# jgkellymit/GENIE-SMEM

Hardware: AMD Instinct MI355X
Metric: query-bases/sec SMEM discovery, 100kb ref x 150bp reads; bit-exact SMEM set (higher is better)
Workload: dtype u8/int32 (2-bit packed bases, int32 SA rows; f64 only in the RMI predict)

## Files before the change

### genie-smem_amd/csrc/kernels.hip

```cpp
#include <hip/hip_runtime.h>

#include <algorithm>
#include <cstdio>
#include <cstdlib>
#include <mutex>
#include <string>
#include <unordered_map>

#include "genie_internal.h"

namespace genie {

namespace {

constexpr int kWave = 64;

__device__ __forceinline__ int rfl(int v) { return __builtin_amdgcn_readfirstlane(v); }
__device__ __forceinline__ void set_wave_priority(int i)
{
    switch (i & 3) {
    case 0: __builtin_amdgcn_s_setprio(0); break;
    case 1: __builtin_amdgcn_s_setprio(1); break;
    case 2: __builtin_amdgcn_s_setprio(2); break;
    default: __builtin_amdgcn_s_setprio(3); break;
// ... 647 lines not shown
    int64_t at = 0;
    template <class T> void take(T *&piece, int64_t bytes)
    {
        piece = base ? reinterpret_cast<T *>(base + at) : nullptr;
        at += ws_align(bytes);
    }
};

template <class F>
inline long long pass_size(long long lo, long long total, F fits)
{
    long long hi = std::max(lo, total);
    while (lo < hi) {
        const long long mid = lo + (hi - lo + 1) / 2;
        if (fits(mid)) lo = mid; else hi = mid - 1;
    }
    return std::min(lo, total);
}

inline int64_t block_sums_bytes(int64_t N) { return (N / 16 + 3) * 8; }

inline int64_t workspace_layout(uint8_t *base, int64_t N, const Geometry &g, Workspace *ws, int64_t vlens_n = 0)
{
    Carver c{base};
    c.take(ws->fwd, N * (int64_t)g.fwd_stride);
    c.take(ws->qp, N * (int64_t)g.qp_stride * 16);
    c.take(ws->status, N * 4);
    c.take(ws->kj, N * (int64_t)g.kj_row * (g.wide ? 4 : 2));
    c.take(ws->counts, N * 4);
    c.take(ws->scan_tmp, block_sums_bytes(N));
    c.take(ws->vlens, vlens_n * 4);
    return c.at + 256;
}

inline int carve_workspace(void *d_ws, int64_t ws_bytes, int64_t N, const Geometry &g, Workspace *ws, int64_t vlens_n = 0)
{
    if (!d_ws || ws_bytes < workspace_layout(static_cast<uint8_t *>(d_ws), N, g, ws, vlens_n) || (reinterpret_cast<uintptr_t>(d_ws) & 255) != 0)
        return GENIE_E_CAPACITY;
    return GENIE_OK;
}

constexpr long long kLongTwoLaneReads = 32768;

struct FindRequest : FindBatch {
    int32_t *counts = nullptr, *slots = nullptr;
    int32_t cap = 0;
    int64_t *offsets = nullptr;
    int32_t *rows = nullptr;
    int64_t cap_rows = 0;
    bool packed = false;
    int row_bytes = 8;
    uint8_t *counts8 = nullptr, *status8 = nullptr;
    int64_t *escapes = nullptr;
    int64_t cap_escapes = 0;
    bool both = false;

    explicit FindRequest(const FindBatch &b) : FindBatch(b) {}
};

constexpr int kLdsBytes = 160 * 1024;
std::mutex g_lds_mu;
std::unordered_map<const void *, int> g_lds_limit;

template <class Kernel>
int allow_large_lds(Kernel k)
{
    const void *fn = reinterpret_cast<const void *>(k);
    int limit;
    {
        std::lock_guard<std::mutex> lk(g_lds_mu);
        auto it = g_lds_limit.find(fn);
        if (it == g_lds_limit.end()) {
            hipFuncAttributes attr;
            HIP_TRY(hipFuncGetAttributes(&attr, fn));
            it = g_lds_limit.emplace(fn, kLdsBytes - (int)attr.sharedSizeBytes).first;
        }
        limit = it->second;
    }
    HIP_TRY(hipFuncSetAttribute(fn, hipFuncAttributeMaxDynamicSharedMemorySize, limit));
    return GENIE_OK;
}

template <class Kernel, class... Args>
int launch_match_table(Kernel km, const Geometry &g, hipStream_t s, Args... args)
{
    if (int rc = allow_large_lds(km)) return rc;
    LAUNCH(km, dim3(g.grid), dim3(g.block), g.lds, s, args...);
    return GENIE_OK;
}

template <int MODE, bool WIDE>
int launch_pipeline(const genie_index *ix, const Geometry &g, const FindRequest &r, const Workspace &ws, hipStream_t s)
{
    int32_t *st = r.status ? r.status : ws.status;
    int32_t *cnt = r.counts ? r.counts : ws.counts;
    const bool c16 = (ix->dev.flags & kFlagCompactTable) != 0;
    const long long mtab_bytes = table_bytes(ix);
    const int cus = ix->num_cus > 0 ? ix->num_cus : 256;
    const int max_len = std::max(g.max_len, 1);
    const int long_flags = ix->opt_search_all | ix->opt_scheduling << 16, flags = long_flags | ix->opt_debug << 8;
    if (ix->ev_search_begin) HIP_TRY(hipEventRecord((hipEvent_t)ix->ev_search_begin, s));
    int rc;
    if (WIDE && r.both)
        rc = launch_match_table(c16 ? match_table_long_both_kernel<true> : match_table_long_both_kernel<false>, g, s, ix->dev,
                                (int)MODE, r.reads, r.lens, (long long)r.N, r.stride, r.fixed_len, reinterpret_cast<uint8_t *>(ws.fwd),
                                g.fwd_stride, ws.qp, g.qp_recs, st, max_len, mtab_bytes, long_flags, cus, ws.vlens);
    else if (WIDE)
        rc = launch_match_table(c16 ? match_table_long_kernel<true> : match_table_long_kernel<false>, g, s, ix->dev, (int)MODE,
                                r.reads, r.lens, (long long)r.N, r.stride, r.fixed_len, reinterpret_cast<uint8_t *>(ws.fwd),
                                g.fwd_stride, ws.qp, g.qp_recs, st, max_len, mtab_bytes, long_flags, cus);
    else if (r.both)
        rc = launch_match_table(c16 ? (g.wps == 4 ? match_table_both_kernel<4, true> : match_table_both_kernel<6, true>)
                                    : (g.wps == 4 ? match_table_both_kernel<4, false> : match_table_both_kernel<8, false>),
                                g, s, ix->dev, (int)MODE, r.reads, r.lens, (long long)r.N, r.stride, r.fixed_len,
                                reinterpret_cast<uint8_t *>(ws.fwd), g.fwd_stride, ws.qp, g.qp_recs, g.qp_stride, st, g.grp,
                                max_len, mtab_bytes, flags, cus, ws.vlens);
    else
        rc = launch_match_table(r.packed ? (c16 ? (g.wps == 4 ? match_table_kernel<4, true, true> : match_table_kernel<6, true, true>)
                                                : (g.wps == 4 ? match_table_kernel<4, false, true> : match_table_kernel<8, false, true>))
                                         : (c16 ? (g.wps == 4 ? match_table_kernel<4, true, false> : match_table_kernel<6, true, false>)
                                                : (g.wps == 4 ? match_table_kernel<4, false, false> : match_table_kernel<8, false, false>)),
                                g, s, ix->dev, (int)MODE, r.reads, r.lens, (long long)r.N, r.stride, r.fixed_len,
                                reinterpret_cast<uint8_t *>(ws.fwd), g.fwd_stride, ws.qp, g.qp_recs, g.qp_stride, st, g.grp,
                                max_len, mtab_bytes, flags, cus);
    if (rc) return rc;
    if (ix->ev_search_end) HIP_TRY(hipEventRecord((hipEvent_t)ix->ev_search_end, s));
    if (ix->opt_search_only) return GENIE_W_SEARCH_ONLY;
    const long long N = r.N;
    const int32_t *lens = r.both && r.lens ? ws.vlens : r.lens;
    uint8_t *head = WIDE ? ws.kj : reinterpret_cast<uint8_t *>(ws.qp) + g.qp_recs * 16;
    const int head_stride = WIDE ? g.kj_row * 4 : g.qp_stride * 16;
    const int tb = 256;
    int reads_per_block = tb;
    unsigned long long *bsums = r.offsets ? reinterpret_cast<unsigned long long *>(ws.scan_tmp) : nullptr;
    if (WIDE) {
        const int lanes = N >= kLongTwoLaneReads ? 2 : 16;
        auto kl = lanes == 2 ? traverse_long_kernel<MODE, 2, 8> : traverse_long_kernel<MODE, 16, 1>;
        LAUNCH(kl, dim3((unsigned)((N + tb / lanes - 1) / (tb / lanes))), dim3(tb), lanes == 2 ? (tb / lanes) * kLongRowBytes : 0, s, lens,
               N, r.fixed_len, r.min_len, ws.fwd, g.fwd_stride, cnt, reinterpret_cast<uint32_t *>(ws.kj),
               g.kj_row, r.offsets ? g.kj_row : r.cap, st, bsums);
        reads_per_block = tb / lanes;
    } else {
        auto kb = traverse_kernel<MODE>;
        const int lds_b = tb * g.fwd_lds;
        if ((rc = allow_large_lds(kb))) return rc;
        LAUNCH(kb, dim3((unsigned)((N + tb - 1) / tb)), dim3(tb), lds_b, s, ix->dev, lens, N,
               r.fixed_len, r.min_len, ws.fwd, g.fwd_stride, g.fwd_lds, cnt, ws.kj, g.kj_row, head, head_stride,
               r.offsets ? g.kj_row : r.cap, st, bsums, r.counts8, r.status8);
    }
    int block_shift = 0;
    while ((1 << block_shift) < reads_per_block) block_shift++;
    if (r.offsets)
        LAUNCH(scan_block_sums_kernel, dim3(1), dim3(kScanBlock), 0, s, bsums, (N + reads_per_block - 1) / reads_per_block);
    long long grid_c = (long long)cus * (32 / kIvWaves);
    const long long need_c = (N + kIvWaves * 4 * kIvUnroll - 1) / (kIvWaves * 4 * kIvUnroll);
    if (grid_c > need_c) grid_c = need_c;
    RowEscapes esc{nullptr, nullptr, 0};
    const int sched_c = ((ix->opt_scheduling >> 2) & 1) | cus << 8;
    if (r.packed) {
        esc.count = reinterpret_cast<unsigned long long *>(r.offsets) + 1;
        esc.list = reinterpret_cast<long long *>(r.escapes);
        esc.cap = r.cap_escapes;
        HIP_TRY(hipMemsetAsync(r.offsets, 0, 16, s));
    }
    auto kc = r.packed ? (r.row_bytes == 6 ? (c16 ? interval_kernel<true, false, true, 2> : interval_kernel<true, false, false, 2>)
                                           : (c16 ? interval_kernel<true, false, true, 1> : interval_kernel<true, false, false, 1>))
            : r.offsets ? (c16 ? interval_kernel<true, WIDE, true> : interval_kernel<true, WIDE, false>)
                        : (c16 ? interval_kernel<false, WIDE, true> : interval_kernel<false, WIDE, false>);
    LAUNCH(kc, dim3((unsigned)grid_c), dim3(kIvWaves * kWave), 0, s, ix->dev, N, ws.kj, g.kj_row, head, head_stride, ws.qp,
           g.qp_stride, r.offsets ? reinterpret_cast<void *>(r.rows) : reinterpret_cast<void *>(r.slots), r.offsets ? 0 : r.cap,
           reinterpret_cast<long long *>(r.offsets), r.offsets ? (long long)r.cap_rows : 0ll, bsums, r.offsets ? cnt : nullptr,
           r.offsets ? block_shift : 0, esc, sched_c);
    return GENIE_OK;
}

template <int MODE>
int launch_find_mode(const genie_index *ix, const Geometry &g, const FindRequest &r, hipStream_t s)
{
    Workspace ws;
    int rc = carve_workspace(r.ws, r.ws_bytes, r.N, g, &ws, r.both ? r.N : 0);
    if (rc) return rc;
    if (g.wide) return launch_pipeline<MODE, true>(ix, g, r, ws, s);
    return launch_pipeline<MODE, false>(ix, g, r, ws, s);
}

}

void set_hip_error(const char *what, int code)
{
    std::lock_guard<std::mutex> lk(g_err_mu);
    g_err = std::string(what) + ": " + hipGetErrorString((hipError_t)code);
}

const char *last_hip_error()
{
    std::lock_guard<std::mutex> lk(g_err_mu);
    return g_err.c_str();
}

int find_smems_geometry(const genie_index *ix, int32_t mode, int32_t max_len, int32_t *grid, int32_t *block,
                        int32_t *lds_bytes)
{
    Geometry g;
    int rc = plan_find_smems(ix, mode, max_len, 1ll << 40, &g);
    if (rc) return rc;
    if (grid) *grid = g.grid;
    if (block) *block = g.block;
    if (lds_bytes) *lds_bytes = g.lds;
    return GENIE_OK;
}

int search_kernel_name(const genie_index *ix, int32_t mode, int32_t max_len, char *buf, int32_t cap)
{
    Geometry g;
    int rc = plan_find_smems(ix, mode, max_len, 1ll << 40, &g);
    if (rc) return rc;
    const std::string c16 = (ix->dev.flags & kFlagCompactTable) ? "true" : "false";
    const std::string name = g.wide ? "match_table_long_kernel<" + c16 + ">"
                                    : "match_table_kernel<" + std::to_string(g.wps) + ", " + c16 + ", false>";
    if (!buf || cap < (int)name.size() + 1) return GENIE_E_CAPACITY;
    memcpy(buf, name.c_str(), name.size() + 1);
    return GENIE_OK;
}

int64_t find_smems_workspace_bytes(int64_t N, int32_t max_len)
{
    Geometry g;
    shape_for(max_len, &g);
    Workspace ws;
    return workspace_layout(nullptr, N, g, &ws);
}

void find_smems_workspace_rows(int32_t max_len, int32_t out[4])
{
    Geometry g;
    shape_for(max_len, &g);
    out[0] = g.fwd_stride;
    out[1] = g.qp_recs;
    out[2] = 0;
    out[3] = g.kj_row * (g.wide ? 4 : 2);
}

static int launch_find_any(const genie_index *ix, int32_t mode, const FindRequest &r, void *stream)
{
    hipStream_t s = (hipStream_t)stream;
    if (r.N == 0) {
        if (r.offsets) HIP_TRY(hipMemsetAsync(r.offsets, 0, r.packed ? 16 : 8, s));
        return GENIE_OK;
    }
    Geometry g;
    int rc = plan_find_smems(ix, mode, r.fixed_len, r.N, &g);
    if (rc) return rc;
    switch (mode) {
    case GENIE_MODE_BWA: return launch_find_mode<GENIE_MODE_BWA>(ix, g, r, s);
    case GENIE_MODE_LUT: return launch_find_mode<GENIE_MODE_LUT>(ix, g, r, s);
    case GENIE_MODE_RMI: return launch_find_mode<GENIE_MODE_RMI>(ix, g, r, s);
    }
    return GENIE_E_INVALID;
}

int launch_find_smems(const genie_index *ix, int32_t mode, const FindBatch &b, int32_t *d_counts, int32_t *d_slots, int32_t cap,
                      void *stream)
{
    FindRequest r(b);
    r.counts = d_counts;
    r.slots = d_slots;
    r.cap = cap;
    return launch_find_any(ix, mode, r, stream);
}

int launch_find_smems_csr(const genie_index *ix, int32_t mode, const FindBatch &b, int64_t *d_offsets, int32_t *d_rows,
                          int64_t out_cap_rows, void *stream)
{
    FindRequest r(b);
    r.offsets = d_offsets;
    r.rows = d_rows;
    r.cap_rows = out_cap_rows;
    return launch_find_any(ix, mode, r, stream);
}

int64_t find_smems_both_workspace_bytes(int64_t N, int32_t max_len)
{
    Geometry g;
    shape_for(max_len, &g);
    Workspace ws;
    return workspace_layout(nullptr, 2 * N, g, &ws, 2 * N);
}

int launch_find_smems_both(const genie_index *ix, int32_t mode, const FindBatch &b, int64_t *d_offsets, int32_t *d_rows,
                           int64_t out_cap_rows, void *stream)
{
    FindRequest r(b);
    r.N = 2 * b.N;
    r.offsets = d_offsets;
    r.rows = d_rows;
    r.cap_rows = out_cap_rows;
    r.both = true;
    return launch_find_any(ix, mode, r, stream);
}

int launch_find_smems_packed(const genie_index *ix, int32_t mode, const FindBatch &b, uint8_t *d_counts8, uint8_t *d_status8,
                             void *d_rows8, int64_t out_cap_rows, int64_t *d_totals, int64_t *d_escapes, int64_t cap_escapes,
                             void *stream, int row_bytes)
{
    FindRequest r(b);
    r.offsets = d_totals;
    r.rows = reinterpret_cast<int32_t *>(d_rows8);
    r.cap_rows = out_cap_rows;
    r.packed = true;
    r.row_bytes = row_bytes;
    r.counts8 = d_counts8;
    r.status8 = d_status8;
    r.escapes = d_escapes;
    r.cap_escapes = cap_escapes;
    return launch_find_any(ix, mode, r, stream);
}

int launch_sa_interval(const genie_index *ix, const uint8_t *d_pats, const int32_t *d_lens, int64_t N, int32_t stride,
                       int32_t fixed_len, int32_t *d_out, void *stream)
{
// ... 218 lines not shown
```

### genie-smem_amd/csrc/short_read_kernel.inc

```

template <bool WIDE>
struct ReadTraits {
    typedef uint8_t fwd_t;
    static constexpr int kj_bits = 16, kj_shift = 8;
};
template <>
struct ReadTraits<true> {
    typedef uint16_t fwd_t;
    static constexpr int kj_bits = 32, kj_shift = 16;
};


typedef unsigned short kb_us2 __attribute__((ext_vector_type(2)));
__device__ __forceinline__ uint32_t kb_pk_max(uint32_t a, uint32_t b)
{
    return __builtin_bit_cast(uint32_t, __builtin_elementwise_max(__builtin_bit_cast(kb_us2, a), __builtin_bit_cast(kb_us2, b)));
}

constexpr int kPairHeadWords = 4;

__device__ __forceinline__ int block_exclusive_scan(int v, int &total)
{
    __shared__ int wave_total[16];
    const int lane = threadIdx.x & (kWave - 1), wave = threadIdx.x >> 6;
// ... 175 lines not shown
    constexpr int kShift = ReadTraits<true>::kj_shift;
    const int lane = threadIdx.x & (kWave - 1), sub = lane & (G - 1);
    const long long r = (long long)blockIdx.x * (blockDim.x / G) + (threadIdx.x / G);
    const bool valid = r < N;
    int st = valid ? status[r] : GENIE_READ_OK;
    const int L = valid ? (lens ? lens[r] : fixed_len) : 0;
    const uint16_t *fw = reinterpret_cast<const uint16_t *>(fwd_in + (valid ? r : 0) * (long long)fwd_stride);
    uint32_t *row = kj_out + (valid ? r : 0) * (long long)kj_stride;
    int i = 0, cnt = 0;
    uint32_t mine = 0;
    bool go = valid && st == GENIE_READ_OK && L > 0;
    int kprev = -1;
    while (__any(go)) {
        uint32_t best = 0;
        int top = i;
        bool more = go;
        if (V == 8) {
            int ctop = i >> 3;
            const uint32_t reach = ((uint32_t)i << 16) | 0xFFFFu;
            bool first = true;
            const int need_lo = (kprev + 1) & ~7;
            const bool fits = go && i - need_lo < kLongWin;
            const bool reload = fits && !(need_lo >= wb && i < wb + kLongWin);
            if (__any(reload)) {
                if (reload) {
                    wb = need_lo;
                    uint4 t[kLongWin / 8 / G];
#pragma unroll
                    for (int u = 0; u < kLongWin / 8 / G; u++) {
                        const int c = (wb >> 3) + sub + G * u;
                        t[u] = c < row_chunks ? *reinterpret_cast<const uint4 *>(fw + 8 * c) : make_uint4(0, 0, 0, 0);
                    }
#pragma unroll
                    for (int u = 0; u < kLongWin / 8 / G; u++) *reinterpret_cast<uint4 *>(wrow + 16 * (sub + G * u)) = t[u];
                }
                wave_lds_fence();
            }
            while (__any(more)) {
                const int c = ctop - sub;
                const bool inb = more && c >= 0;
                uint4 q = make_uint4(0, 0, 0, 0);
                if (inb) {
                    if (fits && 8 * c >= wb) q = *reinterpret_cast<const uint4 *>(wrow + 2 * (8 * c - wb));
                    else q = *reinterpret_cast<const uint4 *>(fw + 8 * c);
                }
                uint32_t qd[4] = {q.x, q.y, q.z, q.w};
                if (first) {
                    const int jmax = (sub == 0) ? (i & 7) : 7;
#pragma unroll
                    for (int d = 0; d < 4; d++) qd[d] &= jmax >= 2 * d + 1 ? 0xFFFFFFFFu : (jmax >= 2 * d ? 0x0000FFFFu : 0u);
                    first = false;
                }
                const uint32_t c0 = (uint32_t)(0xFFFF - 8 * c) - ((uint32_t)(8 * c) << 16);
                uint32_t kmax = 0;
#pragma unroll
                for (int j = 0; j < 8; j++) {
                    const uint32_t vh = (j & 1) ? (qd[j >> 1] & 0xFFFF0000u) : (qd[j >> 1] << 16);
                    const uint32_t key = vh > reach ? vh + (c0 - (uint32_t)j * 0x10001u) : 0u;
                    kmax = max(kmax, key);
                }
                best = max(best, group_max<G>(kmax));
                const bool low = inb && (qd[0] << 16) > reach;
                ctop -= G;
                more = more && ((__ballot(low) >> (lane | (G - 1))) & 1ull);
            }
        }
        while (V == 1 && __any(more)) {
            const int k = top - sub;
            const bool in = more && k > kprev;
            const int v = in ? (int)fw[k] : 0;
            const bool covers = in && v > i;
            const uint32_t key = covers ? ((uint32_t)(v - k) << 16) | (uint32_t)(0xFFFF - k) : 0u;
            best = max(best, group_max<G>(key));
            top -= G;
            more = more && ((__ballot(covers) >> (lane | (G - 1))) & 1ull);
        }
        if (go) {
            const int blen = (int)(best >> 16), bk = 0xFFFF - (int)(best & 0xFFFFu);
            if (blen == 0) { st = GENIE_READ_ABSENT_BASE; go = false; }
            else {
                if (MODE != GENIE_MODE_BWA || blen >= min_len) {
                    const int s_ = cnt + 1;
                    if (sub == (s_ & (G - 1))) mine = (uint32_t)(bk | ((bk + blen) << kShift));
                    if ((s_ & (G - 1)) == G - 1) {
                        const int idx = (s_ & ~(G - 1)) + sub;
                        if (idx > 0) row[idx] = mine;
                    }
                    cnt++;
                }
                kprev = bk;
                i = bk + blen;
                go = i < L;
            }
        }
    }
    if (valid) {
        if (st != GENIE_READ_OK) cnt = 0;
        else {
            const int idx = ((cnt + 1) & ~(G - 1)) + sub;
            if (((cnt + 1) & (G - 1)) != 0 && idx >= 1 && idx <= cnt) row[idx] = mine;
            if (cnt > cap) st = GENIE_READ_OVERFLOW;
        }
        if (sub == 0) {
            row[0] = (uint32_t)cnt;
            status[r] = st;
        }
    }
    if (block_sums) {
        int total;
        const int before = block_exclusive_scan(valid && sub == 0 ? cnt : 0, total);
        if (valid && sub == 0) counts[r] = before;
        if (threadIdx.x == 0) block_sums[blockIdx.x] = (unsigned long long)total;
    } else if (valid && sub == 0) {
        counts[r] = cnt;
    }
}

constexpr int kIvWaves = 8;
constexpr int kIvUnroll = 1;
constexpr int kIvList = 128;

struct RowEscapes {
    unsigned long long *count;
    long long *list;
    long long cap;
};
template <int COUT>
__device__ __forceinline__ void emit_row(void *out, long long idx, int k, int j, int lo, int hi, const RowEscapes &esc)
{
    if (COUT == 0) {
        store_nt(reinterpret_cast<int4 *>(out) + idx, make_uint4((uint32_t)k, (uint32_t)j, (uint32_t)lo, (uint32_t)hi));
        return;
    }
    constexpr uint32_t kTop = COUT == 1 ? 0xFFFFu : 0xFFu;
    uint32_t span = (uint32_t)(hi - lo);
    if (span >= kTop) {
        const unsigned long long slot = atomicAdd(esc.count, 1ull);
        if ((long long)slot < esc.cap) {
            esc.list[2 * slot] = idx;
            esc.list[2 * slot + 1] = hi;
        }
        span = kTop;
    }
    if (COUT == 1) {
        reinterpret_cast<uint2 *>(out)[idx] = make_uint2((uint32_t)k | (uint32_t)j << 8 | span << 16, (uint32_t)lo);
    } else {
        uint16_t *o = reinterpret_cast<uint16_t *>(out) + 3 * idx;
        o[0] = (uint16_t)((uint32_t)k | (uint32_t)j << 8);
        o[1] = (uint16_t)lo;
        o[2] = (uint16_t)(((uint32_t)lo >> 16) | span << 8);
    }
}

template <bool CSR, bool WIDE, bool C16, int COUT = 0>
__global__ void __launch_bounds__(kIvWaves * 64, 8) interval_kernel(DevIndex ix, long long N,
                                                                    const void *__restrict__ kj_in, int kj_stride,
                                                                    const uint8_t *__restrict__ head_in, int head_stride,
                                                                    const RefRec *__restrict__ qp_in, int qp_stride,
                                                                    void *__restrict__ out, int cap,
                                                                    long long *__restrict__ offsets, long long out_cap,
                                                                    const unsigned long long *__restrict__ block_base,
                                                                    const int32_t *__restrict__ before_in_block, int block_shift,
                                                                    RowEscapes esc, int sched)
{
    __shared__ int4 lists[kIvWaves][kIvList];
    typedef typename std::conditional<WIDE, uint32_t, uint16_t>::type kj_t;
    typedef typename std::conditional<WIDE, QRecs, QPlain>::type QIn;
    constexpr int kHeadEntries = kPairHeadWords * 8 / (int)sizeof(kj_t);
    const int lane = threadIdx.x & (kWave - 1);
    const int wave = rfl((int)(threadIdx.x >> 6));
    const int sub = lane & 15;
    const int P2 = ix.P2;
    const __amdgpu_buffer_rsrc_t ov =
        __builtin_amdgcn_make_buffer_rsrc(const_cast<MatchOv16 *>(ix.ov), 0, ix.ov_entries * (int)sizeof(MatchOv16), 0x00020000);
    int4 *list = lists[wave];
    int nlist = 0;
    auto search_list = [&](int o, int n) {
        if (lane < n) {
            const int4 en = list[o + lane];
            const int k = en.w & 0xFFFF, j = (int)((uint32_t)en.w >> 16);
            const QIn qp{reinterpret_cast<decltype(QIn::p)>(qp_in + (long long)en.z * qp_stride)};
            const int2 iv = sa_interval(ix, ix.dir, qp, k, j - k);
            emit_row<COUT>(out, ((long long)en.y << 32) | (uint32_t)en.x, k, j, iv.x, iv.y, esc);
        }
    };
    constexpr int U = kIvUnroll;
    const long long step = (long long)gridDim.x * kIvWaves * 4 * U;
    const bool rotate = !(sched & 1);
    const int round_of_block = (int)(blockIdx.x / (uint32_t)(sched >> 8));
    int it = round_of_block;
    for (long long r0 = ((long long)blockIdx.x * kIvWaves + wave) * 4 * U; r0 < N; r0 += step, it++) {
        if (rotate) set_wave_priority(it);
        long long r[U], base[U];
        int c[U];
        bool more = false;
#pragma unroll
        for (int u = 0; u < U; u++) {
            r[u] = r0 + 4 * u + (lane >> 4);
            const bool have = r[u] < N;
            if (!have) r[u] = 0;
            c[u] = have ? (int)reinterpret_cast<const kj_t *>(head_in + r[u] * (long long)head_stride)[0] : 0;
            base[u] = CSR ? (have ? (long long)block_base[r[u] >> block_shift] + before_in_block[r[u]] : 0) : r[u] * (long long)cap;
            if (CSR && have && sub == 0) {
                if (!COUT) offsets[r[u]] = base[u];
                if (r[u] == N - 1) offsets[COUT ? 0 : N] = base[u] + c[u];
            }
            if (!CSR) c[u] = c[u] < cap ? c[u] : cap;
            more |= c[u] > 0;
        }
        for (int t0 = 0; __any(more); t0 += 16) {
            const int t = t0 + sub;
            uint32_t e[U];
            uint64_t w[U];
            int4 ra[U], rb[U];
            bool act[U];
            more = false;
#pragma unroll
            for (int u = 0; u < U; u++) {
                act[u] = t < c[u] && (!CSR || base[u] + t < out_cap);
                more |= t0 + 16 < c[u];
                const kj_t *row = t + 1 < kHeadEntries ? reinterpret_cast<const kj_t *>(head_in + r[u] * (long long)head_stride)
                                                       : reinterpret_cast<const kj_t *>(kj_in) + r[u] * (long long)kj_stride;
                e[u] = act[u] ? (uint32_t)row[t + 1] : 0u;
            }
#pragma unroll
            for (int u = 0; u < U; u++) {
                const int k = (int)(e[u] & ((1u << ReadTraits<WIDE>::kj_shift) - 1));
                w[u] = act[u] ? QIn{reinterpret_cast<decltype(QIn::p)>(qp_in + r[u] * (long long)qp_stride)}.win(k) : 0ull;
            }
#pragma unroll
            for (int u = 0; u < U; u++) {
                const uint32_t c = (uint32_t)(w[u] >> (64 - 2 * P2));
                const int4 *en = C16 ? reinterpret_cast<const int4 *>(reinterpret_cast<const MatchRec16 *>(ix.mtab) + c)
                                     : reinterpret_cast<const int4 *>(ix.mtab + c);
                ra[u] = make_int4(0, 0, 0, 0);
                rb[u] = make_int4(0, 0, 0, 0);
                if (act[u]) { ra[u] = en[0]; if (!C16) rb[u] = en[1]; }
            }
#pragma unroll
            for (int u = 0; u < U; u++) {
                const int k = (int)(e[u] & ((1u << ReadTraits<WIDE>::kj_shift) - 1)), j = (int)(e[u] >> ReadTraits<WIDE>::kj_shift);
                const int len = j - k;
                const uint32_t meta = (uint32_t)ra[u].x;
                bool fast = false;
                int2 iv = make_int2(-1, -1);
                if (C16) {
                    const uint32_t cnt4 = (meta >> 24) & 15u, nib = meta >> 28, lb = meta & 0xFFFFFFu;
                    if (act[u] && cnt4 == 0) {
                        if (len == (int)nib) { fast = true; iv = make_int2((int)lb, ra[u].y); }
                    } else if (act[u] && (nib & kM16Wide) && cnt4 <= 3u && len >= P2) {
                        const uint32_t xk = (uint32_t)((w[u] << (2 * P2)) >> 32);
                        const int cl = len - P2 < 16 ? len - P2 : 16;
                        const uint32_t km = cl == 0 ? 0u : ~0u << (32 - 2 * cl);
                        const uint32_t bits = (((((uint32_t)ra[u].y ^ xk) & km) == 0 ? 1u : 0u) | ((((uint32_t)ra[u].z ^ xk) & km) == 0 ? 2u : 0u) |
                                               ((((uint32_t)ra[u].w ^ xk) & km) == 0 ? 4u : 0u)) & ((1u << cnt4) - 1u);
                        fast = len <= P2 + 16 || __popc(bits) == 1;
                        if (bits) {
                            const int first = (int)lb + __ffs((int)bits) - 1;
                            iv = make_int2(first, first + __popc(bits) - 1);
                        }
                    } else if (act[u] && (cnt4 == kM16More || !(nib & kM16General)) && len >= P2) {
                        const uint32_t total = cnt4 == kM16More ? 7u + nib : cnt4;
                        const uint32_t xk16 = (uint32_t)((w[u] << (2 * P2)) >> 48);
                        const int cl = len - P2 < 8 ? len - P2 : 8;
                        const uint32_t km16 = cl == 0 ? 0u : (0xFFFFu << (16 - 2 * cl)) & 0xFFFFu;
                        const uint32_t k16[6] = {(uint32_t)ra[u].y & 0xFFFFu, (uint32_t)ra[u].y >> 16, (uint32_t)ra[u].z & 0xFFFFu,
                                                 (uint32_t)ra[u].z >> 16, (uint32_t)ra[u].w & 0xFFFFu, (uint32_t)ra[u].w >> 16};
                        const uint32_t ninl = cnt4 == kM16More ? (uint32_t)kM16Keys - 1u : cnt4;
                        uint32_t bits = 0, xm = 0xFFFFu;
#pragma unroll
                        for (int i = 0; i < kM16Keys; i++) bits |= (((k16[i] ^ xk16) & km16) == 0 && (uint32_t)i < ninl) ? 1u << i : 0u;
                        if (cnt4 == kM16More) mt_ov_scan(ov, k16[5], (int)total - (kM16Keys - 1), xk16, km16, xm, bits);
                        fast = len <= P2 + 8 || __popc(bits) == 1;
                        if (bits) {
                            const int first = (int)lb + __ffs((int)bits) - 1;
                            iv = make_int2(first, first + __popc(bits) - 1);
                        }
                    }
                } else if (act[u] && !(meta & kMatchSlow)) {
                    const uint32_t rows = meta >> 24;
                    if (rows == 0) {
                        if (len == (int)(meta & 0xFFu)) { fast = true; iv = make_int2(ra[u].y, ra[u].z); }
                    } else if (len >= P2) {
                        const uint32_t xk = (uint32_t)((w[u] << (2 * P2)) >> 32);
                        const int cl = len - P2 < 16 ? len - P2 : 16;
                        const uint32_t km = cl == 0 ? 0u : ~0u << (32 - 2 * cl);
                        uint32_t bits = ((((uint32_t)ra[u].z ^ xk) & km) == 0 ? 1u : 0u) | ((((uint32_t)ra[u].w ^ xk) & km) == 0 ? 2u : 0u) |
                                        ((((uint32_t)rb[u].x ^ xk) & km) == 0 ? 4u : 0u) | ((((uint32_t)rb[u].y ^ xk) & km) == 0 ? 8u : 0u) |
                                        ((((uint32_t)rb[u].z ^ xk) & km) == 0 ? 16u : 0u) | ((((uint32_t)rb[u].w ^ xk) & km) == 0 ? 32u : 0u);
                        bits &= (1u << rows) - 1u;
                        fast = len <= P2 + 16 || __popc(bits) == 1;
                        if (bits) {
                            const int first = (int)ra[u].y + __ffs((int)bits) - 1;
                            iv = make_int2(first, first + __popc(bits) - 1);
                        }
                    }
                }
                if (fast) emit_row<COUT>(out, base[u] + t, k, j, iv.x, iv.y, esc);
                const bool general = act[u] && !fast;
                const unsigned long long gb = __ballot(general);
                if (gb) {
                    if (general) {
                        const long long row = base[u] + t;
                        list[nlist + __popcll(gb & ((1ull << lane) - 1ull))] = make_int4((int)(uint32_t)row, (int)(row >> 32), (int)r[u], k | (j << 16));
                    }
                    nlist += __popcll(gb);
                    wave_lds_fence();
                    if (nlist >= 64) {
                        nlist -= 64;
                        search_list(nlist, 64);
                        wave_lds_fence();
                    }
                }
            }
        }
    }
    if (nlist) search_list(0, nlist);
}
```

Measured before the change: 197.4 billion.

## Add tiled row-parallel interval kernel staging query records in LDS for CSR output

For short reads with CSR row output, a new interval_rows_kernel replaces interval_kernel. It stages a tile of reads' packed query records into LDS, then assigns one lane per output row using a binary search over per-read row starts, rather than iterating per read with per-lane unrolled loops. The aim is better load balance across lanes and coalesced loading of query data, which should reduce divergence and idle lanes when reads have different SMEM counts. The fast-path match logic is factored into a shared helper. The new path adds dynamic LDS per block, which may reduce occupancy, and adds block-wide syncs per tile.

```diff
diff --git a/genie-smem_amd/csrc/kernels.hip b/genie-smem_amd/csrc/kernels.hip
--- a/genie-smem_amd/csrc/kernels.hip
+++ b/genie-smem_amd/csrc/kernels.hip
@@ -823,9 +823,6 @@
     while ((1 << block_shift) < reads_per_block) block_shift++;
     if (r.offsets)
         LAUNCH(scan_block_sums_kernel, dim3(1), dim3(kScanBlock), 0, s, bsums, (N + reads_per_block - 1) / reads_per_block);
-    long long grid_c = (long long)cus * (32 / kIvWaves);
-    const long long need_c = (N + kIvWaves * 4 * kIvUnroll - 1) / (kIvWaves * 4 * kIvUnroll);
-    if (grid_c > need_c) grid_c = need_c;
     RowEscapes esc{nullptr, nullptr, 0};
     const int sched_c = ((ix->opt_scheduling >> 2) & 1) | cus << 8;
     if (r.packed) {
@@ -834,9 +831,24 @@
         esc.cap = r.cap_escapes;
         HIP_TRY(hipMemsetAsync(r.offsets, 0, 16, s));
     }
-    auto kc = r.packed ? (r.row_bytes == 6 ? (c16 ? interval_kernel<true, false, true, 2> : interval_kernel<true, false, false, 2>)
-                                           : (c16 ? interval_kernel<true, false, true, 1> : interval_kernel<true, false, false, 1>))
-            : r.offsets ? (c16 ? interval_kernel<true, WIDE, true> : interval_kernel<true, WIDE, false>)
+    if (!WIDE && r.offsets) {
+        const int lds_c = kIvTile * g.qp_stride * 16;
+        auto kr = r.packed ? (r.row_bytes == 6 ? (c16 ? interval_rows_kernel<true, 2> : interval_rows_kernel<false, 2>)
+                                               : (c16 ? interval_rows_kernel<true, 1> : interval_rows_kernel<false, 1>))
+                           : (c16 ? interval_rows_kernel<true, 0> : interval_rows_kernel<false, 0>);
+        const int bpc = std::max(1, std::min(32 / kIvWaves, kLdsBytes / (lds_c + kIvRowsStaticLds)));
+        const long long grid_r = std::min((long long)cus * bpc, (N + kIvTile - 1) / kIvTile);
+        const long long rounds = (N + grid_r * kIvTile - 1) / (grid_r * kIvTile);
+        const int tile_reads = (int)((N + grid_r * rounds - 1) / (grid_r * rounds));
+        LAUNCH(kr, dim3((unsigned)grid_r), dim3(kIvWaves * kWave), lds_c, s, ix->dev, N, reinterpret_cast<const uint16_t *>(ws.kj),
+               g.kj_row, ws.qp, g.qp_stride, g.qp_recs, reinterpret_cast<void *>(r.rows), reinterpret_cast<long long *>(r.offsets),
+               (long long)r.cap_rows, bsums, cnt, block_shift, esc, sched_c, tile_reads);
+        return GENIE_OK;
+    }
+    long long grid_c = (long long)cus * (32 / kIvWaves);
+    const long long need_c = (N + kIvWaves * 4 * kIvUnroll - 1) / (kIvWaves * 4 * kIvUnroll);
+    if (grid_c > need_c) grid_c = need_c;
+    auto kc = r.offsets ? (c16 ? interval_kernel<true, true, true> : interval_kernel<true, true, false>)
                         : (c16 ? interval_kernel<false, WIDE, true> : interval_kernel<false, WIDE, false>);
     LAUNCH(kc, dim3((unsigned)grid_c), dim3(kIvWaves * kWave), 0, s, ix->dev, N, ws.kj, g.kj_row, head, head_stride, ws.qp,
            g.qp_stride, r.offsets ? reinterpret_cast<void *>(r.rows) : reinterpret_cast<void *>(r.slots), r.offsets ? 0 : r.cap,
diff --git a/genie-smem_amd/csrc/short_read_kernel.inc b/genie-smem_amd/csrc/short_read_kernel.inc
--- a/genie-smem_amd/csrc/short_read_kernel.inc
+++ b/genie-smem_amd/csrc/short_read_kernel.inc
@@ -351,7 +351,69 @@
     }
 }
 
-template <bool CSR, bool WIDE, bool C16, int COUT = 0>
+template <bool C16>
+__device__ __forceinline__ bool interval_from_entry(const int4 ra, const int4 rb, uint64_t w, int len, int P2,
+                                                    const __amdgpu_buffer_rsrc_t ov, bool act, int2 &iv)
+{
+    const uint32_t meta = (uint32_t)ra.x;
+    bool fast = false;
+    iv = make_int2(-1, -1);
+    if (C16) {
+        const uint32_t cnt4 = (meta >> 24) & 15u, nib = meta >> 28, lb = meta & 0xFFFFFFu;
+        if (act && cnt4 == 0) {
+            if (len == (int)nib) { fast = true; iv = make_int2((int)lb, ra.y); }
+        } else if (act && (nib & kM16Wide) && cnt4 <= 3u && len >= P2) {
+            const uint32_t xk = (uint32_t)((w << (2 * P2)) >> 32);
+            const int cl = len - P2 < 16 ? len - P2 : 16;
+            const uint32_t km = cl == 0 ? 0u : ~0u << (32 - 2 * cl);
+            const uint32_t bits = (((((uint32_t)ra.y ^ xk) & km) == 0 ? 1u : 0u) | ((((uint32_t)ra.z ^ xk) & km) == 0 ? 2u : 0u) |
+                                   ((((uint32_t)ra.w ^ xk) & km) == 0 ? 4u : 0u)) & ((1u << cnt4) - 1u);
+            fast = len <= P2 + 16 || __popc(bits) == 1;
+            if (bits) {
+                const int first = (int)lb + __ffs((int)bits) - 1;
+                iv = make_int2(first, first + __popc(bits) - 1);
+            }
+        } else if (act && (cnt4 == kM16More || !(nib & kM16General)) && len >= P2) {
+            const uint32_t total = cnt4 == kM16More ? 7u + nib : cnt4;
+            const uint32_t xk16 = (uint32_t)((w << (2 * P2)) >> 48);
+            const int cl = len - P2 < 8 ? len - P2 : 8;
+            const uint32_t km16 = cl == 0 ? 0u : (0xFFFFu << (16 - 2 * cl)) & 0xFFFFu;
+            const uint32_t k16[6] = {(uint32_t)ra.y & 0xFFFFu, (uint32_t)ra.y >> 16, (uint32_t)ra.z & 0xFFFFu,
+                                     (uint32_t)ra.z >> 16, (uint32_t)ra.w & 0xFFFFu, (uint32_t)ra.w >> 16};
+            const uint32_t ninl = cnt4 == kM16More ? (uint32_t)kM16Keys - 1u : cnt4;
+            uint32_t bits = 0, xm = 0xFFFFu;
+#pragma unroll
+            for (int i = 0; i < kM16Keys; i++) bits |= (((k16[i] ^ xk16) & km16) == 0 && (uint32_t)i < ninl) ? 1u << i : 0u;
+            if (cnt4 == kM16More) mt_ov_scan(ov, k16[5], (int)total - (kM16Keys - 1), xk16, km16, xm, bits);
+            fast = len <= P2 + 8 || __popc(bits) == 1;
+            if (bits) {
+                const int first = (int)lb + __ffs((int)bits) - 1;
+                iv = make_int2(first, first + __popc(bits) - 1);
+            }
+        }
+    } else if (act && !(meta & kMatchSlow)) {
+        const uint32_t rows = meta >> 24;
+        if (rows == 0) {
+            if (len == (int)(meta & 0xFFu)) { fast = true; iv = make_int2(ra.y, ra.z); }
+        } else if (len >= P2) {
+            const uint32_t xk = (uint32_t)((w << (2 * P2)) >> 32);
+            const int cl = len - P2 < 16 ? len - P2 : 16;
+            const uint32_t km = cl == 0 ? 0u : ~0u << (32 - 2 * cl);
+            uint32_t bits = ((((uint32_t)ra.z ^ xk) & km) == 0 ? 1u : 0u) | ((((uint32_t)ra.w ^ xk) & km) == 0 ? 2u : 0u) |
+                            ((((uint32_t)rb.x ^ xk) & km) == 0 ? 4u : 0u) | ((((uint32_t)rb.y ^ xk) & km) == 0 ? 8u : 0u) |
+                            ((((uint32_t)rb.z ^ xk) & km) == 0 ? 16u : 0u) | ((((uint32_t)rb.w ^ xk) & km) == 0 ? 32u : 0u);
+            bits &= (1u << rows) - 1u;
+            fast = len <= P2 + 16 || __popc(bits) == 1;
+            if (bits) {
+                const int first = (int)ra.y + __ffs((int)bits) - 1;
+                iv = make_int2(first, first + __popc(bits) - 1);
+            }
+        }
+    }
+    return fast;
+}
+
+template <bool CSR, bool WIDE, bool C16>
 __global__ void __launch_bounds__(kIvWaves * 64, 8) interval_kernel(DevIndex ix, long long N,
                                                                     const void *__restrict__ kj_in, int kj_stride,
                                                                     const uint8_t *__restrict__ head_in, int head_stride,
@@ -362,6 +424,8 @@
                                                                     const int32_t *__restrict__ before_in_block, int block_shift,
                                                                     RowEscapes esc, int sched)
 {
+    static_assert(WIDE || !CSR, "short reads, CSR rows: interval_rows_kernel");
+    constexpr int COUT = 0;
     __shared__ int4 lists[kIvWaves][kIvList];
     typedef typename std::conditional<WIDE, uint32_t, uint16_t>::type kj_t;
     typedef typename std::conditional<WIDE, QRecs, QPlain>::type QIn;
@@ -440,61 +504,8 @@
             for (int u = 0; u < U; u++) {
                 const int k = (int)(e[u] & ((1u << ReadTraits<WIDE>::kj_shift) - 1)), j = (int)(e[u] >> ReadTraits<WIDE>::kj_shift);
                 const int len = j - k;
-                const uint32_t meta = (uint32_t)ra[u].x;
-                bool fast = false;
-                int2 iv = make_int2(-1, -1);
-                if (C16) {
-                    const uint32_t cnt4 = (meta >> 24) & 15u, nib = meta >> 28, lb = meta & 0xFFFFFFu;
-                    if (act[u] && cnt4 == 0) {
-                        if (len == (int)nib) { fast = true; iv = make_int2((int)lb, ra[u].y); }
-                    } else if (act[u] && (nib & kM16Wide) && cnt4 <= 3u && len >= P2) {
-                        const uint32_t xk = (uint32_t)((w[u] << (2 * P2)) >> 32);
-                        const int cl = len - P2 < 16 ? len - P2 : 16;
-                        const uint32_t km = cl == 0 ? 0u : ~0u << (32 - 2 * cl);
-                        const uint32_t bits = (((((uint32_t)ra[u].y ^ xk) & km) == 0 ? 1u : 0u) | ((((uint32_t)ra[u].z ^ xk) & km) == 0 ? 2u : 0u) |
-                                               ((((uint32_t)ra[u].w ^ xk) & km) == 0 ? 4u : 0u)) & ((1u << cnt4) - 1u);
-                        fast = len <= P2 + 16 || __popc(bits) == 1;
-                        if (bits) {
-                            const int first = (int)lb + __ffs((int)bits) - 1;
-                            iv = make_int2(first, first + __popc(bits) - 1);
-                        }
-                    } else if (act[u] && (cnt4 == kM16More || !(nib & kM16General)) && len >= P2) {
-                        const uint32_t total = cnt4 == kM16More ? 7u + nib : cnt4;
-                        const uint32_t xk16 = (uint32_t)((w[u] << (2 * P2)) >> 48);
-                        const int cl = len - P2 < 8 ? len - P2 : 8;
-                        const uint32_t km16 = cl == 0 ? 0u : (0xFFFFu << (16 - 2 * cl)) & 0xFFFFu;
-                        const uint32_t k16[6] = {(uint32_t)ra[u].y & 0xFFFFu, (uint32_t)ra[u].y >> 16, (uint32_t)ra[u].z & 0xFFFFu,
-                                                 (uint32_t)ra[u].z >> 16, (uint32_t)ra[u].w & 0xFFFFu, (uint32_t)ra[u].w >> 16};
-                        const uint32_t ninl = cnt4 == kM16More ? (uint32_t)kM16Keys - 1u : cnt4;
-                        uint32_t bits = 0, xm = 0xFFFFu;
-#pragma unroll
-                        for (int i = 0; i < kM16Keys; i++) bits |= (((k16[i] ^ xk16) & km16) == 0 && (uint32_t)i < ninl) ? 1u << i : 0u;
-                        if (cnt4 == kM16More) mt_ov_scan(ov, k16[5], (int)total - (kM16Keys - 1), xk16, km16, xm, bits);
-                        fast = len <= P2 + 8 || __popc(bits) == 1;
-                        if (bits) {
-                            const int first = (int)lb + __ffs((int)bits) - 1;
-                            iv = make_int2(first, first + __popc(bits) - 1);
-                        }
-                    }
-                } else if (act[u] && !(meta & kMatchSlow)) {
-                    const uint32_t rows = meta >> 24;
-                    if (rows == 0) {
-                        if (len == (int)(meta & 0xFFu)) { fast = true; iv = make_int2(ra[u].y, ra[u].z); }
-                    } else if (len >= P2) {
-                        const uint32_t xk = (uint32_t)((w[u] << (2 * P2)) >> 32);
-                        const int cl = len - P2 < 16 ? len - P2 : 16;
-                        const uint32_t km = cl == 0 ? 0u : ~0u << (32 - 2 * cl);
-                        uint32_t bits = ((((uint32_t)ra[u].z ^ xk) & km) == 0 ? 1u : 0u) | ((((uint32_t)ra[u].w ^ xk) & km) == 0 ? 2u : 0u) |
-                                        ((((uint32_t)rb[u].x ^ xk) & km) == 0 ? 4u : 0u) | ((((uint32_t)rb[u].y ^ xk) & km) == 0 ? 8u : 0u) |
-                                        ((((uint32_t)rb[u].z ^ xk) & km) == 0 ? 16u : 0u) | ((((uint32_t)rb[u].w ^ xk) & km) == 0 ? 32u : 0u);
-                        bits &= (1u << rows) - 1u;
-                        fast = len <= P2 + 16 || __popc(bits) == 1;
-                        if (bits) {
-                            const int first = (int)ra[u].y + __ffs((int)bits) - 1;
-                            iv = make_int2(first, first + __popc(bits) - 1);
-                        }
-                    }
-                }
+                int2 iv;
+                const bool fast = interval_from_entry<C16>(ra[u], rb[u], w[u], len, P2, ov, act[u], iv);
                 if (fast) emit_row<COUT>(out, base[u] + t, k, j, iv.x, iv.y, esc);
                 const bool general = act[u] && !fast;
                 const unsigned long long gb = __ballot(general);
@@ -516,3 +527,132 @@
     }
     if (nlist) search_list(0, nlist);
 }
+
+constexpr int kIvTile = 256;
+constexpr int kIvChunks = kIvTile * 255 / kWave + 2;
+constexpr int kIvRowsStaticLds = kIvWaves * kIvList * 16 + 2 * kIvTile * 4 + ((kIvChunks + 15) & ~15) + 16;
+
+template <bool C16, int COUT>
+__global__ void __launch_bounds__(kIvWaves * 64, 8) interval_rows_kernel(DevIndex ix, long long N,
+                                                                         const uint16_t *__restrict__ kj_in, int kj_stride,
+                                                                         const RefRec *__restrict__ qp_in, int qp_stride, int qp_recs,
+                                                                         void *__restrict__ out,
+                                                                         long long *__restrict__ offsets, long long out_cap,
+                                                                         const unsigned long long *__restrict__ block_base,
+                                                                         const int32_t *__restrict__ before_in_block, int block_shift,
+                                                                         RowEscapes esc, int sched, int tile_reads)
+{
+    extern __shared__ __align__(16) uint8_t smem[];
+    __shared__ int4 lists[kIvWaves][kIvList];
+    __shared__ int starts[2 * kIvTile];
+    __shared__ uint8_t chunk_read[kIvChunks];
+    __shared__ int tile_rows;
+    constexpr int kHeadEntries = kPairHeadWords * 8 / 2;
+    const int lane = threadIdx.x & (kWave - 1);
+    const int wave = rfl((int)(threadIdx.x >> 6));
+    const int P2 = ix.P2;
+    const int slot_bytes = qp_stride * 16, head_off = qp_recs * 16;
+    const __amdgpu_buffer_rsrc_t ov =
+        __builtin_amdgcn_make_buffer_rsrc(const_cast<MatchOv16 *>(ix.ov), 0, ix.ov_entries * (int)sizeof(MatchOv16), 0x00020000);
+    int4 *list = lists[wave];
+    int nlist = 0;
+    auto search_list = [&](int o, int n) {
+        if (lane < n) {
+            const int4 en = list[o + lane];
+            const int k = en.w & 0xFFFF, j = (int)((uint32_t)en.w >> 16);
+            const QPlain qp{reinterpret_cast<const uint64_t *>(qp_in + (long long)en.z * qp_stride)};
+            const int2 iv = sa_interval(ix, ix.dir, qp, k, j - k);
+            emit_row<COUT>(out, ((long long)en.y << 32) | (uint32_t)en.x, k, j, iv.x, iv.y, esc);
+        }
+    };
+    const bool rotate = !(sched & 1);
+    int it = (int)(blockIdx.x / (uint32_t)(sched >> 8));
+    const long long tiles = (N + tile_reads - 1) / tile_reads;
+    if ((int)threadIdx.x < kIvTile) starts[kIvTile + threadIdx.x] = 0x7FFFFFFF;
+    for (long long tile = blockIdx.x; tile < tiles; tile += gridDim.x, it++) {
+        if (rotate) set_wave_priority(it);
+        const long long r0 = tile * tile_reads;
+        const int reads = (int)(N - r0 < (long long)tile_reads ? N - r0 : (long long)tile_reads);
+        const long long tile_base = (long long)block_base[r0 >> block_shift] + before_in_block[r0];
+        const bool have = (int)threadIdx.x < reads;
+        const long long r = r0 + (have ? (int)threadIdx.x : 0);
+        const long long base = have ? (long long)block_base[r >> block_shift] + before_in_block[r] : 0;
+        {
+            const uint4 *src = reinterpret_cast<const uint4 *>(qp_in + r0 * (long long)qp_stride);
+            uint4 *dst = reinterpret_cast<uint4 *>(smem);
+            const int units = reads * qp_stride;
+            constexpr int kInFlight = 4;
+            for (int e0 = threadIdx.x; e0 < units; e0 += kInFlight * kIvWaves * kWave) {
+                uint4 v[kInFlight];
+#pragma unroll
+                for (int u = 0; u < kInFlight; u++) {
+                    const int e = e0 + u * kIvWaves * kWave;
+                    v[u] = e < units ? src[e] : make_uint4(0, 0, 0, 0);
+                }
+#pragma unroll
+                for (int u = 0; u < kInFlight; u++) {
+                    const int e = e0 + u * kIvWaves * kWave;
+                    if (e < units) dst[e] = v[u];
+                }
+            }
+        }
+        __syncthreads();
+        if ((int)threadIdx.x < kIvTile) {
+            const int c = have ? (int)*reinterpret_cast<const uint16_t *>(smem + threadIdx.x * slot_bytes + head_off) : 0;
+            if (have) {
+                if (!COUT) offsets[r] = base;
+                if (r == N - 1) offsets[COUT ? 0 : N] = base + c;
+            }
+            const int first = have ? (int)(base - tile_base) : 0x7FFFFFFF;
+            starts[threadIdx.x] = first;
+            if (have)
+                for (int ch = (first + kWave - 1) >> 6; (ch << 6) < first + c; ch++) chunk_read[ch] = (uint8_t)threadIdx.x;
+            if (have && (int)threadIdx.x == reads - 1) {
+                tile_rows = first + c;
+                chunk_read[(first + c + kWave - 1) >> 6] = (uint8_t)threadIdx.x;
+            }
+        }
+        __syncthreads();
+        const int total = tile_rows;
+        for (int q0 = wave * kWave; q0 < total && tile_base + q0 < out_cap; q0 += kIvWaves * kWave) {
+            const int q = q0 + lane;
+            const bool act = q < total && tile_base + q < out_cap;
+            const int lo = rfl((int)chunk_read[q0 >> 6]), span = rfl((int)chunk_read[(q0 >> 6) + 1]) - lo;
+            int i = lo;
+            for (int s = span > 0 ? 1 << (31 - __builtin_clz(span)) : 0; s > 0; s >>= 1) i += starts[i + s] <= q ? s : 0;
+            const int t = act ? q - starts[i] : 0;
+            const uint8_t *slot = smem + i * slot_bytes;
+            uint32_t e = 0;
+            if (act) e = t + 1 < kHeadEntries ? (uint32_t)reinterpret_cast<const uint16_t *>(slot + head_off)[t + 1]
+                                              : (uint32_t)kj_in[(r0 + i) * (long long)kj_stride + t + 1];
+            const int k = (int)(e & 0xFFu), j = (int)(e >> 8);
+            const uint64_t *wp = reinterpret_cast<const uint64_t *>(slot) + (k >> 5);
+            const uint64_t w = act ? funnel(wp[0], wp[1], (k & 31) * 2) : 0ull;
+            const uint32_t c = (uint32_t)(w >> (64 - 2 * P2));
+            const int4 *en = C16 ? reinterpret_cast<const int4 *>(reinterpret_cast<const MatchRec16 *>(ix.mtab) + c)
+                                 : reinterpret_cast<const int4 *>(ix.mtab + c);
+            int4 ra = make_int4(0, 0, 0, 0), rb = make_int4(0, 0, 0, 0);
+            if (act) { ra = en[0]; if (!C16) rb = en[1]; }
+            int2 iv;
+            const bool fast = interval_from_entry<C16>(ra, rb, w, j - k, P2, ov, act, iv);
+            if (fast) emit_row<COUT>(out, tile_base + q, k, j, iv.x, iv.y, esc);
+            const bool general = act && !fast;
+            const unsigned long long gb = __ballot(general);
+            if (gb) {
+                if (general) {
+                    const long long row = tile_base + q;
+                    list[nlist + __popcll(gb & ((1ull << lane) - 1ull))] = make_int4((int)(uint32_t)row, (int)(row >> 32), (int)(r0 + i), k | (j << 16));
+                }
+                nlist += __popcll(gb);
+                wave_lds_fence();
+                if (nlist >= 64) {
+                    nlist -= 64;
+                    search_list(nlist, 64);
+                    wave_lds_fence();
+                }
+            }
+        }
+        __syncthreads();
+    }
+    if (nlist) search_list(0, nlist);
+}
```

Result: faster. 204.9 billion (median of 6 runs) (+3.8%).
